# yharby/flac-raster

Measured on NVIDIA B200. Metric: encode GSamples/s (streaming tiles -> FLAC frames; decode GSamples/s reported beside it), higher is better.
Workload: dtype int32

## Files before the change

### flac_raster_b200/csrc/frb_encode.cuh

```cuda
#pragma once
#include "frb_common.cuh"

namespace frb {

constexpr int kEncThreads = 256;
constexpr int kSPT = 16;
constexpr int kMaxBlock = kEncThreads * kSPT;
constexpr int kMaxOrd = 12;
constexpr int kMaxPO = 8;
#define PX(i) ((i) + ((uint32_t)(i) >> 4))
constexpr int kBufWords = kMaxBlock + kMaxBlock / 16;

struct EncSrc {
    const void *audio;
    uint32_t a16;
};
__device__ __forceinline__ const void *audio_at(const EncSrc &S, int64_t idx) {
    return reinterpret_cast<const uint8_t *>(S.audio) + idx * (S.a16 ? 2 : 4);
}
struct TaskLoc {
    uint32_t n, a16;
    const void *src;
};
__device__ __forceinline__ int32_t sample_at(const TaskLoc &L, uint32_t i) {
// ... 1218 lines not shown
        if (h_n_samples[i] == 0) return FRB_ERR_INVALID_ARG;
        EncStreamDev d;
        d.n_samples = h_n_samples[i]; d.audio_base = h_audio_base[i]; d.out_offset = 0;
        d.sample_rate = h_sample_rate[i]; d.frame_base = (uint32_t)frames;
        d.n_frames = (uint32_t)((h_n_samples[i] + p->blocksize - 1) / p->blocksize); d.pad = 0;
        frames += d.n_frames;
        hs[i] = d;
    }
    if (frames == 0 || frames * p->channels > 0x7FFFFFFFull) return FRB_ERR_INVALID_ARG;
    EncWorkspace w;
    if (enc_ws_layout(p, frames, d_workspace, &w) > workspace_bytes) return FRB_ERR_OVERFLOW;
    cudaStream_t s = (cudaStream_t)stream;
    static thread_local std::vector<float> win;
    static thread_local uint32_t win_bs = 0, win_n = 0;
    if (win_bs != p->blocksize || win_n != (uint32_t)level_cfg(p->level).windows) {
        win.assign(FRB_MAX_BLOCKSIZE, 1.0f);
        make_tukey(win.data(), (int)p->blocksize, 0.5f / (float)level_cfg(p->level).windows);
        win_bs = p->blocksize; win_n = (uint32_t)level_cfg(p->level).windows;
    }
    const bool ms = enc_mid_side(p);
    const uint32_t an_ch = ms ? 4u : p->channels;
    std::vector<EncStreamDev> vhs;
    if (ms) {
        vhs = hs;
        uint64_t cum = 0;
        for (uint32_t i = 0; i < p->n_streams; i++) { vhs[i].audio_base = (int64_t)(4 * cum); cum += hs[i].n_samples; }
        if (cum > frames * (uint64_t)p->blocksize) return FRB_ERR_INVALID_ARG;
        FRB_TRY(small_upload(w.vstreams, vhs.data(), sizeof(EncStreamDev) * vhs.size(), s));
    }
    FRB_TRY(small_upload(w.streams, hs.data(), sizeof(EncStreamDev) * hs.size(), s));
    FRB_TRY(small_upload(w.window, win.data(), sizeof(float) * FRB_MAX_BLOCKSIZE, s));
    FRB_TRY(small_fill(w.err_flag, 0u, 256, s));
    const std::vector<EncStreamDev> &ahs = ms ? vhs : hs;
    const EncStreamDev *an_streams = ms ? w.vstreams : w.streams;
    const bool a16 = (p->reserved & 1u) != 0;
    if (a16 && p->bps != 16) return FRB_ERR_INVALID_ARG;
    const EncSrc in_audio = {d_audio, a16 ? 1u : 0u};
    const EncSrc an_audio = ms ? EncSrc{w.vaudio, 0u} : in_audio;
    const uint32_t an_esz = an_audio.a16 ? 2u : 4u;
    const uint32_t side_ch = ms ? 3u : 0xFFFFFFFFu;
    uint32_t *sub_est = ms ? w.sub_est : nullptr;
    if (ms) {
        uint64_t max_n = 0;
        for (uint32_t i = 0; i < p->n_streams; i++) max_n = std::max<uint64_t>(max_n, hs[i].n_samples);
        uint32_t gx = (uint32_t)std::min<uint64_t>((max_n + 256 * 8 - 1) / (256 * 8), std::max<uint32_t>(1u, (uint32_t)kNumSMs * 16 / p->n_streams));
        if (gx < 1) gx = 1;
        k_ms_expand<<<gx * p->n_streams, 256, 0, s>>>(w.streams, w.vstreams, in_audio, w.vaudio, gx, w.err_flag);
        FRB_LAUNCH_CHECK("k_ms_expand");
    }
    const uint32_t slot_words = slot_words_for(p->blocksize, enc_slot_bps(p));
    static bool attr_set[64] = {false};
    if (first_call_on_device(attr_set)) {
        FRB_CUDA(cudaFuncSetAttribute(k_encode_subframes, cudaFuncAttributeMaxDynamicSharedMemorySize, (int)sizeof(EncShared)));
        cudaFuncSetAttribute(k_enc_code<false>, cudaFuncAttributePreferredSharedMemoryCarveout, 20);
        cudaFuncSetAttribute(k_enc_stats<false, 9>, cudaFuncAttributePreferredSharedMemoryCarveout, 5);
        cudaFuncSetAttribute(k_enc_stats<false, 13>, cudaFuncAttributePreferredSharedMemoryCarveout, 5);
        cudaFuncSetAttribute(k_enc_stats<false, 0>, cudaFuncAttributePreferredSharedMemoryCarveout, 5);
        cudaGetLastError();
    }
    const LevelCfg cfg = level_cfg(p->level);
    const bool fast = p->blocksize == (uint32_t)kMaxBlock && cfg.max_po >= 3 && cfg.max_po <= 6;
    std::vector<uint32_t> slow;
    const uint32_t total_tasks = (uint32_t)(frames * an_ch);
    if (fast) {
        const uint64_t base_addr = (uint64_t)reinterpret_cast<uintptr_t>(an_audio.audio);
        if (base_addr & (an_esz - 1)) return FRB_ERR_INVALID_ARG;
        for (uint32_t i = 0; i < p->n_streams; i++) {
            const EncStreamDev &d = ahs[i];
            const bool tail = (d.n_samples % p->blocksize) != 0;
            for (uint32_t c = 0; c < an_ch; c++) {
                const bool aligned = ((base_addr + ((uint64_t)d.audio_base + (uint64_t)c * d.n_samples) * an_esz) & (an_esz == 2 ? 7u : 15u)) == 0;
                for (uint32_t k = aligned ? (tail ? d.n_frames - 1 : d.n_frames) : 0; k < d.n_frames; k++)
                    slow.push_back((d.frame_base + k) * an_ch + c);
            }
        }
        if (!slow.empty()) {
            if (4 * slow.size() <= (1u << 20)) FRB_TRY(small_upload(w.slow_tasks, slow.data(), 4 * slow.size(), s));
            else {
                FRB_CUDA(cudaMemcpyAsync(w.slow_tasks, slow.data(), 4 * slow.size(), cudaMemcpyHostToDevice, s));
                FRB_CUDA(cudaStreamSynchronize(s));
            }
        }
    }
    k_frame_table<<<(uint32_t)((frames + 255) / 256), 256, 0, s>>>(an_streams, p->n_streams, p->blocksize, (uint32_t)frames, w.frame_table);
    FRB_LAUNCH_CHECK("k_frame_table");
    prof_begin(6, s);
    if (fast && slow.size() < total_tasks) {
        const uint32_t windows = (uint32_t)cfg.windows, max_lpc = (uint32_t)cfg.max_lpc_order;
        const uint32_t n_cands = max_lpc == 0 ? 0u : windows == 1 ? 1u : windows == 2 ? 3u : 9u;
        const bool wide = p->bps > 16;
        const dim3 grid((uint32_t)frames, ms ? 3u : p->channels), grid_side((uint32_t)frames, 1);
        prof_begin(4, s);
#define FRB_STATS(W, NL, G, C0, EX) k_enc_stats<W, NL><<<G, kEncThreads, 0, s>>>(w.frame_table, an_ch, p->bps, windows, (uint32_t)cfg.max_po, an_audio, \
            w.window, w.stats, w.autoc, w.fx_fin, C0, EX)
#define FRB_STATS_L(NL) do { if (wide) FRB_STATS(true, NL, grid, 0u, 0u); else FRB_STATS(false, NL, grid, 0u, 0u); \
                             if (ms) FRB_STATS(true, NL, grid_side, 3u, 1u); } while (0)
        if (max_lpc == 0) FRB_STATS_L(0);
        else if (max_lpc <= 8) FRB_STATS_L(9);
        else FRB_STATS_L(13);
#undef FRB_STATS_L
#undef FRB_STATS
        prof_end(4, s);
        FRB_LAUNCH_CHECK("k_enc_stats");
        k_enc_fixed<<<(total_tasks + 3) / 4, 128, 0, s>>>(w.frame_table, an_ch, p->bps, (uint32_t)cfg.max_po, total_tasks, an_audio,
                                                        w.stats, w.fx_fin, side_ch);
        FRB_LAUNCH_CHECK("k_enc_fixed");
        const uint32_t n_slots = n_cands;
        const uint32_t model_threads = total_tasks * n_slots;
        if (n_cands) {
#define FRB_MODEL(MO) k_enc_model<MO><<<(model_threads + 127) / 128, 128, 0, s>>>(w.frame_table, an_ch, p->bps, \
            p->blocksize, windows, max_lpc, n_slots, total_tasks, an_audio, w.stats, w.autoc, w.cands, side_ch)
        if (max_lpc <= 8) FRB_MODEL(8); else FRB_MODEL(12);
#undef FRB_MODEL
        FRB_LAUNCH_CHECK("k_enc_model");
        }
        prof_begin(0, s);
#define FRB_CODE(W, G, C0, EX) k_enc_code<W><<<G, kEncThreads, 0, s>>>(w.frame_table, an_ch, p->bps, (uint32_t)cfg.max_po, n_cands, an_audio, \
            w.stats, w.cands, slot_words, w.slots, w.sub_bits, C0, EX, sub_est)
        if (wide) FRB_CODE(true, grid, 0u, 0u); else FRB_CODE(false, grid, 0u, 0u);
        if (ms) FRB_CODE(true, grid_side, 3u, 1u);
#undef FRB_CODE
        prof_end(0, s);
        FRB_LAUNCH_CHECK("k_enc_code");
    }
    if (!fast || !slow.empty()) {
        const uint32_t grid = fast ? (uint32_t)slow.size() : total_tasks;
        k_encode_subframes<<<grid, kEncThreads, sizeof(EncShared), s>>>(
            an_streams, p->n_streams, an_ch, p->bps, p->blocksize, p->level, an_audio, w.window, slot_words, w.slots, w.sub_bits,
            fast ? w.slow_tasks : nullptr, side_ch, sub_est);
        FRB_LAUNCH_CHECK("k_encode_subframes");
    }
    prof_end(6, s);
    if (ms) {
        k_ms_choose<<<(uint32_t)((frames + 255) / 256), 256, 0, s>>>(w.streams, p->n_streams, p->blocksize, (uint32_t)frames,
                                                                   (uint32_t)cfg.loose, w.sub_est, w.frame_sel);
        FRB_LAUNCH_CHECK("k_ms_choose");
    }
    k_frame_sizes<<<(uint32_t)((frames + 255) / 256), 256, 0, s>>>(w.streams, p->n_streams, p->channels, p->blocksize,
                                                                 (uint32_t)frames, w.sub_bits, w.frame_bytes, an_ch, ms ? w.frame_sel : nullptr);
    FRB_LAUNCH_CHECK("k_frame_sizes");
    t_last_analyse.ws = d_workspace; t_last_analyse.frames = frames; t_last_analyse.n_streams = p->n_streams;
    k_stream_scan<<<p->n_streams, 1024, 0, s>>>(w.streams, w.frame_bytes, w.frame_off, w.stream_bytes);
    FRB_LAUNCH_CHECK("k_stream_scan");
    if (d_stream_bytes)
        FRB_CUDA(cudaMemcpyAsync(d_stream_bytes, w.stream_bytes, 8 * (size_t)p->n_streams, cudaMemcpyDeviceToDevice, s));
    if (h_stream_bytes) {
        FRB_TRY(small_download(h_stream_bytes, w.stream_bytes, 8 * (size_t)p->n_streams, s));
    }
    return FRB_OK;
}

extern "C" int frb_encode_emit(const frb_encode_params *p, void *d_workspace, size_t workspace_bytes,
                               const uint64_t *h_out_offset, uint8_t *d_out, size_t out_capacity,
                               uint32_t *d_frame_bytes, void *stream) {
    using namespace frb;
    if (!enc_params_ok(p) || !d_workspace || !d_out) return FRB_ERR_INVALID_ARG;
    cudaStream_t s = (cudaStream_t)stream;
    EncWorkspace w0;
    (void)enc_ws_layout(p, 0, d_workspace, &w0);
    uint64_t frames;
    if (t_last_analyse.ws == d_workspace && t_last_analyse.n_streams == p->n_streams && t_last_analyse.frames) frames = t_last_analyse.frames;
    else {
        EncStreamDev last;
        FRB_TRY(small_download(&last, w0.streams + (p->n_streams - 1), sizeof last, s));
        frames = (uint64_t)last.frame_base + last.n_frames;
    }
    EncWorkspace w;
    if (enc_ws_layout(p, frames, d_workspace, &w) > workspace_bytes) return FRB_ERR_OVERFLOW;
    if (h_out_offset) {
        FRB_TRY(small_upload(w.out_offs, h_out_offset, 8 * (size_t)p->n_streams, s));
        k_set_out_offsets<<<(p->n_streams + 255) / 256, 256, 0, s>>>(w.streams, w.out_offs, p->n_streams);
        FRB_LAUNCH_CHECK("k_set_out_offsets");
    } else {
// ... 50 lines not shown
```

### flac_raster_b200/csrc/frb_encode_fast.cuh

```cuda
#pragma once

constexpr int kMaxSets = 6;
constexpr int kMaxCands = 9;
constexpr int kLags = kMaxOrd + 1;

struct EncSubStats {
    unsigned long long e[5];
    uint32_t wasted, flags;
    uint32_t fx_order, fx_bits, fx_po, fx_bad;
    uint8_t fx_params[64];
};
struct EncCand {
    int32_t type, order, precision, shift;
    int32_t coefs[kMaxOrd];
};

struct FrameDesc {
    int64_t src0;
    uint64_t ns;
    uint32_t n, stream;
};
__global__ void __launch_bounds__(256)
k_frame_table(const EncStreamDev *__restrict__ streams, uint32_t n_streams, uint32_t blocksize, uint32_t total_frames,
              FrameDesc *__restrict__ out) {
// ... 152 lines not shown
        const bool hi = lane >= 16;
        const unsigned long long b_m = __shfl_sync(0xFFFFFFFFu, b, src), mine_m = __shfl_sync(0xFFFFFFFFu, mine, src);
        const uint32_t myl_m = __shfl_sync(0xFFFFFFFFu, myl, src);
        const bool act_m = (uint32_t)src < M, actd_m = act_m && myl_m <= P;
        uint32_t k1 = 0, b1 = 0, k2 = 0, b2 = 0;
        if (act_m) rice_estimate(hi ? b_m : a, (!hi && lane == 0) ? np0 - order : np0, k_limit, &k1, &b1);
        if (hi ? actd_m : act_m) {
            uint32_t np = hi ? (n >> (P - myl_m)) : np1;
            if (hi ? (((uint32_t)src >> (myl_m - 1)) == 0) : (lane == 0)) np -= order;
            rice_estimate(hi ? mine_m : a + b, np, k_limit, &k2, &b2);
        }
        const uint32_t kb_u = __shfl_sync(0xFFFFFFFFu, k1, src + 16), bb_u = __shfl_sync(0xFFFFFFFFu, b1, src + 16);
        const uint32_t kd_u = __shfl_sync(0xFFFFFFFFu, k2, src + 16), bd_u = __shfl_sync(0xFFFFFFFFu, b2, src + 16);
        if (!hi) { ka = k1; ba = b1; kb = kb_u; bb = bb_u; kc = k2; bc = b2; kd = kd_u; bd = bd_u; }
    } else {
        if (act) {
            rice_estimate(a, lane == 0 ? np0 - order : np0, k_limit, &ka, &ba);
            rice_estimate(b, np0, k_limit, &kb, &bb);
            rice_estimate(a + b, lane == 0 ? np1 - order : np1, k_limit, &kc, &bc);
        }
        if (actd) {
            uint32_t np = n >> (P - myl);
            if (((uint32_t)lane >> (myl - 1)) == 0) np -= order;
            rice_estimate(mine, np, k_limit, &kd, &bd);
        }
    }
    unsigned long long tot = warp_sum_u32((ba & 0xFFFFu) + (bb & 0xFFFFu), (ba >> 16) + (bb >> 16)) + 6;
    uint32_t rb = tot > 0xFFFFFFFFull ? 0xFFFFFFFFu : (uint32_t)tot, best_l = 0;
    tot = warp_sum_u32(bc & 0xFFFFu, bc >> 16) + 6;
    { const uint32_t c = tot > 0xFFFFFFFFull ? 0xFFFFFFFFu : (uint32_t)tot; if (c < rb) { rb = c; best_l = 1; } }
#pragma unroll
    for (int l = 2; l <= 6; l++) {
        if ((uint32_t)l <= P) {
            const uint32_t x = (actd && myl == (uint32_t)l) ? bd : 0u;
            tot = warp_sum_u32(x & 0xFFFFu, x >> 16) + 6;
            const uint32_t c = tot > 0xFFFFFFFFull ? 0xFFFFFFFFu : (uint32_t)tot;
            if (c < rb) { rb = c; best_l = (uint32_t)l; }
        }
    }
    if (best_l == 0) { if (act) { params[2 * lane] = (uint8_t)ka; params[2 * lane + 1] = (uint8_t)kb; } }
    else if (best_l == 1) { if (act) params[lane] = (uint8_t)kc; }
    else if (actd && myl == best_l) params[(uint32_t)lane >> (myl - 1)] = (uint8_t)kd;
    *rb_out = rb; *best_l_out = best_l;
}

struct StatsShared {
    uint32_t orv[8], diff[8];
    unsigned long long e[8][5];
    double ac[8][kLags];
};

#ifndef FRB_STATS_MINB
#define FRB_STATS_MINB 4
#endif
#ifndef FRB_CODE_MINB
#define FRB_CODE_MINB 4
#endif
#ifndef FRB_CODE_RELOAD
#define FRB_CODE_RELOAD 1
#endif
#ifndef FRB_STATS_LATEWIN
#define FRB_STATS_LATEWIN 0
#endif
#ifndef FRB_STATS_RELOAD
#define FRB_STATS_RELOAD 1
#endif
template <bool WIDE, int NLAGS>
__global__ void __launch_bounds__(kEncThreads, (NLAGS > 9 || WIDE) ? 2 : FRB_STATS_MINB)
k_enc_stats(const FrameDesc *__restrict__ frames, uint32_t channels, uint32_t bps_stream,
            uint32_t windows, uint32_t max_po_cfg, const EncSrc audio,
            const float *__restrict__ window, EncSubStats *__restrict__ stats, double *__restrict__ autoc_out,
            unsigned long long *__restrict__ fx_fin, uint32_t c0, uint32_t side_extra) {
    __shared__ StatsShared S;
    const uint32_t cch = blockIdx.y + c0, sbps = bps_stream + side_extra;
    const uint32_t task = blockIdx.x * channels + cch;
    const TaskLoc L = locate_task(frames, audio, blockIdx.x, cch);
    if (!fast_eligible(L)) return;
    const int tid = threadIdx.x, lane = tid & 31, warp = tid >> 5;
    constexpr uint32_t n = kMaxBlock;
    constexpr int HALO = NLAGS > 0 ? NLAGS - 1 : 0;
    int32_t xs[28];
    load_samples28(L, tid, xs);
    float wv[kSPT + HALO + 1];
    auto load_window = [&]() {
        if (NLAGS > 0) {
            const float4 *wp = reinterpret_cast<const float4 *>(window + tid * kSPT) - HALO / 4;
#pragma unroll
            for (int q = 0; q < (kSPT + HALO) / 4; q++) {
                float4 v = make_float4(0.f, 0.f, 0.f, 0.f);
                if (tid > 0 || q >= HALO / 4) v = __ldg(wp + q);
                wv[4 * q] = v.x; wv[4 * q + 1] = v.y; wv[4 * q + 2] = v.z; wv[4 * q + 3] = v.w;
            }
        }
    };
#if !FRB_STATS_LATEWIN
    load_window();
#endif
    uint32_t orv = 0, diff = 0;
    const int32_t x_first = sample_at(L, 0);
#pragma unroll
    for (int s = 0; s < kSPT; s++) { orv |= (uint32_t)xs[12 + s]; diff |= (uint32_t)(xs[12 + s] ^ x_first); }
    orv = __reduce_or_sync(0xFFFFFFFFu, orv);
    diff = __reduce_or_sync(0xFFFFFFFFu, diff);
    if (lane == 0) { S.orv[warp] = orv; S.diff[warp] = diff; }
    __syncthreads();
    orv = 0; diff = 0;
#pragma unroll
    for (int w = 0; w < 8; w++) { orv |= S.orv[w]; diff |= S.diff[w]; }
    uint32_t wasted = orv ? (uint32_t)(__ffs((int)orv) - 1) : 0;
    if (wasted > sbps) wasted = sbps;
    if (wasted) {
#pragma unroll
// ... 294 lines not shown
            er = __dadd_rn(er, __ddiv_rn((double)lpv[i], (double)(1 << ns)));
            long long q = llround(er);
            if (q > qmax) q = qmax; else if (q < qmin) q = qmin;
            er = __dsub_rn(er, (double)q); C.coefs[i] = (int32_t)q;
        }
        sh = 0;
    }
    C.type = 3; C.order = (int)order; C.precision = (int)prec; C.shift = sh;
}

template <int MAXO>
__global__ void __launch_bounds__(128)
k_enc_model(const FrameDesc *__restrict__ frames, uint32_t channels, uint32_t bps_stream,
            uint32_t blocksize, uint32_t windows, uint32_t max_lpc_cfg, uint32_t n_cands, uint32_t total_tasks,
            const EncSrc audio, EncSubStats *__restrict__ stats, const double *__restrict__ autoc_in,
            EncCand *__restrict__ cands, uint32_t side_ch) {
    const uint32_t gid = blockIdx.x * blockDim.x + threadIdx.x;
    const uint32_t task = gid / n_cands, slot = gid - task * n_cands;
    if (task >= total_tasks) return;
    const uint32_t f = task / channels;
    const TaskLoc L = locate_task(frames, audio, f, task - f * channels);
    if (!fast_eligible(L)) return;
    constexpr uint32_t n = kMaxBlock;
    EncCand C;
    C.type = 0; C.order = 0; C.precision = 0; C.shift = 0;
#pragma unroll
    for (int j = 0; j < kMaxOrd; j++) C.coefs[j] = 0;
    const EncSubStats *stp = stats + task;
    const uint32_t st_flags = stp->flags;
    const uint32_t bps = bps_stream + (task - f * channels == side_ch ? 1u : 0u) - stp->wasted;
    if (!(st_flags & 1u)) {
        if constexpr (MAXO > 0) {
            uint32_t set = 0;
            bool punch = false;
            if (slot == 0) set = 0;
            else if (slot <= 2) set = slot;
            else { const uint32_t ci = slot - 3; set = 3 + ci / 2; punch = (ci & 1u) != 0; }
            const double *a = autoc_in + ((size_t)task * kMaxSets + set) * kLags;
            double autoc[MAXO + 1];
#pragma unroll
            for (int l = 0; l <= MAXO; l++) autoc[l] = a[l];
            const uint32_t max_lpc = max_lpc_cfg;
            if (punch) {
                const double *root = autoc_in + (size_t)task * kMaxSets * kLags;
#pragma unroll
                for (int l = 0; l < MAXO; l++) if ((uint32_t)l < max_lpc) autoc[l] = root[l] - autoc[l];
            }
            model_one<MAXO>(autoc, max_lpc, n, bps, qlp_precision_for(bps_stream, blocksize), C);
        }
    }
    cands[(size_t)task * kMaxCands + slot] = C;
}

template <bool WIDE>
struct CodeShared {
    uint32_t bitbuf[WIDE ? 4232 : 2052];
    SearchShared search;
    uint8_t best_params[64];
    uint32_t scan[kEncThreads / 32];
};

__device__ __forceinline__ void put_bits_atomic(uint32_t *buf, uint32_t pos, uint32_t v, uint32_t len) {
    const uint32_t o = pos & 31u;
    const unsigned long long x = (unsigned long long)v << (64u - o - len);
    const uint32_t hi = (uint32_t)(x >> 32), lo = (uint32_t)x;
    if (hi) atomicOr(&buf[pos >> 5], hi);
    if (lo) atomicOr(&buf[(pos >> 5) + 1], lo);
}

__device__ __forceinline__ void put_sample_atomic(uint32_t *buf, uint32_t pos, int32_t x, uint32_t bps) {
    if (bps > 32) { put_bits_atomic(buf, pos, x < 0 ? 1u : 0u, bps - 32); put_bits_atomic(buf, pos + bps - 32, (uint32_t)x, 32); }
    else if (bps) put_bits_atomic(buf, pos, (uint32_t)x & (bps == 32 ? 0xFFFFFFFFu : ((1u << bps) - 1u)), bps);
}

struct PackWriter {
    uint32_t addr, fill, hi;
    __device__ __forceinline__ void init(uint32_t *b, uint32_t bitpos) {
        addr = (uint32_t)__cvta_generic_to_shared(b) + ((bitpos >> 5) << 2); fill = bitpos & 31u; hi = 0;
    }
    __device__ __forceinline__ void put(uint32_t v, uint32_t len) {
        const uint32_t vh = v << (32u - len);
        hi |= vh >> fill;
        const uint32_t lo = __funnelshift_lc(0u, vh, 32u - fill);
        fill += len;
        asm volatile("{\n\t.reg .pred p;\n\t"
                     "setp.ge.u32 p, %1, 32;\n\t"
                     "@p red.shared.or.b32 [%2], %0;\n\t"
                     "@p mov.b32 %0, %3;\n\t"
                     "@p add.u32 %2, %2, 4;\n\t"
                     "@p sub.u32 %1, %1, 32;\n\t"
                     "}\n" : "+r"(hi), "+r"(fill), "+r"(addr) : "r"(lo) : "memory");
    }
    __device__ __forceinline__ void put0(uint32_t v, uint32_t len) {
        uint32_t vh;
        asm("shl.b32 %0, %1, %2;" : "=r"(vh) : "r"(v), "r"(32u - len));
        hi |= vh >> fill;
        const uint32_t lo = __funnelshift_lc(0u, vh, 32u - fill);
        fill += len;
        asm volatile("{\n\t.reg .pred p;\n\t"
                     "setp.ge.u32 p, %1, 32;\n\t"
                     "@p red.shared.or.b32 [%2], %0;\n\t"
                     "@p mov.b32 %0, %3;\n\t"
                     "@p add.u32 %2, %2, 4;\n\t"
                     "@p sub.u32 %1, %1, 32;\n\t"
                     "}\n" : "+r"(hi), "+r"(fill), "+r"(addr) : "r"(lo) : "memory");
    }
    __device__ __forceinline__ void zeros(uint32_t q) {
        fill += q;
        while (fill >= 32) {
// ... 15 lines not shown
    const uint32_t kbit = 1u << kcur, kmask = kbit - 1u, k1 = kcur + 1;
#pragma unroll 1
    for (uint32_t s = skip; s < (uint32_t)kSPT; s++) {
        const uint32_t u = (uint32_t)r[s];
        const uint32_t q = u >> kcur;
        const uint32_t tailv = kbit | (u & kmask);
        if (q + k1 <= 32) bw.put(tailv, q + k1);
        else { bw.zeros(q); bw.put(tailv, k1); }
    }
    bw.finish();
}

template <bool WIDE, int TAPS>
__device__ __forceinline__ uint32_t residual16(const int32_t (&xs)[28], const int32_t (&cf)[kMaxOrd], int shift, int32_t (&r)[kSPT],
                                               uint32_t *hi_mismatch) {
    uint32_t ora = 0, bad = 0;
#pragma unroll
    for (int s = 0; s < kSPT; s++) {
        if (WIDE) {
            long long acc = 0;
#pragma unroll
            for (int j = 0; j < TAPS; j++) acc += (long long)cf[j] * (long long)xs[12 + s - 1 - j];
            const long long v = (long long)xs[12 + s] - (acc >> shift);
            r[s] = (int32_t)v;
            bad |= (uint32_t)((int32_t)(v >> 32) ^ (r[s] >> 31));
        } else {
            int32_t acc = 0;
#pragma unroll
            for (int j = 0; j < TAPS; j++) acc += cf[j] * xs[12 + s - 1 - j];
            r[s] = (int32_t)((uint32_t)xs[12 + s] - (uint32_t)(acc >> shift));
        }
        ora |= (uint32_t)abs(r[s]);
    }
    *hi_mismatch = bad;
    return ora;
}

__device__ __noinline__ bool residual_overflows(const void *src, uint32_t a16, uint32_t wasted, const EncCand *__restrict__ C, int tid) {
    const int order = C->order, shift = C->shift;
    TaskLoc L;
    L.src = src; L.a16 = a16; L.n = kMaxBlock;
    bool bad = false;
    for (int s = 0; s < kSPT; s++) {
        const int i = tid * kSPT + s;
        if (i < order) continue;
        long long acc = 0;
        for (int j = 0; j < order; j++) acc += (long long)C->coefs[j] * (long long)(sample_at(L, (uint32_t)(i - 1 - j)) >> wasted);
        const long long v = (long long)(sample_at(L, (uint32_t)i) >> wasted) - (acc >> shift);
        if (v > 2147483647ll || v <= -2147483648ll) bad = true;
    }
    return bad;
}

template <bool WIDE>
__global__ void __launch_bounds__(kEncThreads, WIDE ? 2 : FRB_CODE_MINB)
k_enc_code(const FrameDesc *__restrict__ frames, uint32_t channels, uint32_t bps_stream,
           uint32_t max_po_cfg, uint32_t n_cands, const EncSrc audio,
           const EncSubStats *__restrict__ stats, const EncCand *__restrict__ cands, uint32_t slot_words,
           uint32_t *__restrict__ slots, uint32_t *__restrict__ sub_bits, uint32_t c0, uint32_t side_extra,
           uint32_t *__restrict__ sub_est) {
    __shared__ __align__(16) CodeShared<WIDE> S;
    const uint32_t cch = blockIdx.y + c0;
    const uint32_t task = blockIdx.x * channels + cch;
    const TaskLoc L = locate_task(frames, audio, blockIdx.x, cch);
    if (!fast_eligible(L)) return;
    const int tid = threadIdx.x, lane = tid & 31, warp = tid >> 5;
    constexpr uint32_t n = kMaxBlock;
    const uint32_t k_limit = bps_stream > 16 ? 31u : 15u;
    const EncSubStats *stp = stats + task;
    const uint32_t wasted = stp->wasted, st_flags = stp->flags;
    const uint32_t bps = bps_stream + side_extra - wasted;
    constexpr bool RELOAD = FRB_CODE_RELOAD != 0 && !WIDE;
    int32_t xs0[28];
    if constexpr (!RELOAD) {
        load_samples28(L, tid, xs0);
        if (wasted) {
#pragma unroll
            for (int j = 0; j < 28; j++) xs0[j] >>= wasted;
        }
    }
    {
        constexpr int nq = (int)(sizeof(S.bitbuf) / 16);
        uint4 *b4 = reinterpret_cast<uint4 *>(S.bitbuf);
        for (int q = tid; q < nq; q += kEncThreads) b4[q] = make_uint4(0, 0, 0, 0);
    }
    const uint32_t verbatim_bits = 8 + wasted + n * bps;
    int best_type = 1, best_order = 0, best_prec = 0, best_shift = 0, best_slot = -1, best_po = 0;
    uint32_t best_bits = verbatim_bits;
    int32_t r[kSPT];
    int cur_slot = -1;
    const uint32_t P = max_po_cfg;

    auto eval_residual = [&](const EncCand &C, const EncCand *Cg, bool *bad_out) -> uint32_t {
        int32_t xr[28];
        if constexpr (RELOAD) {
            load_samples28(L, tid, xr);
            if (wasted) {
#pragma unroll
                for (int j = 0; j < 28; j++) xr[j] >>= wasted;
            }
        }
        const int32_t (&xs)[28] = pick_ref<RELOAD>(xr, xs0);
        int32_t cf[kMaxOrd];
#pragma unroll
        for (int j = 0; j < kMaxOrd; j++) cf[j] = C.coefs[j];
        uint32_t ora, him;
        if (C.order <= 4) ora = residual16<WIDE, 4>(xs, cf, C.shift, r, &him);
        else if (C.order <= 8) ora = residual16<WIDE, 8>(xs, cf, C.shift, r, &him);
        else ora = residual16<WIDE, 12>(xs, cf, C.shift, r, &him);
        if (tid == 0) {
            ora = 0;
#pragma unroll
            for (int s = 0; s < kSPT; s++) { if (s < C.order) r[s] = 0; ora |= (uint32_t)abs(r[s]); }
        }
        bool bad = false;
        if (Cg != nullptr && ((WIDE && him) || ora >= 0x40000000u)) bad = residual_overflows(L.src, L.a16, wasted, Cg, tid);
        *bad_out = bad;
        return ora;
    };

    if (st_flags & 1u) {
        const uint32_t b = 8 + wasted + bps;
        if (b < best_bits) { best_type = 0; best_bits = b; }
    } else {
        if ((st_flags & 2u) && stp->fx_bits < best_bits) {
            best_bits = stp->fx_bits; best_type = 2; best_order = (int)stp->fx_order; best_po = (int)stp->fx_po; best_slot = -2;
            if (tid < 64) S.best_params[tid] = stp->fx_params[tid];
        }
        for (uint32_t slot = 0; slot <= n_cands; slot++) {
            const bool final_pass = slot == n_cands;
            const EncCand *Cg = nullptr;
            EncCand C;
            if (!final_pass) {
                Cg = cands + (size_t)task * kMaxCands + slot;
                C = *Cg;
                if (C.type == 0) continue;
            } else {
                if (best_type < 2 || best_slot == cur_slot) break;
                if (best_slot == -2) {
                    C.type = 2; C.order = best_order; C.precision = 0; C.shift = 0;
#pragma unroll
                    for (int j = 0; j < kMaxOrd; j++) C.coefs[j] = 0;
                    if (best_order == 1) { C.coefs[0] = 1; }
                    else if (best_order == 2) { C.coefs[0] = 2; C.coefs[1] = -1; }
                    else if (best_order == 3) { C.coefs[0] = 3; C.coefs[1] = -3; C.coefs[2] = 1; }
                    else if (best_order == 4) { C.coefs[0] = 4; C.coefs[1] = -6; C.coefs[2] = 4; C.coefs[3] = -1; }
                } else {
                    Cg = cands + (size_t)task * kMaxCands + best_slot;
                    C = *Cg;
                }
            }
            bool bad_lane;
            const uint32_t ora = eval_residual(C, Cg, &bad_lane);
            if (final_pass) break;
            cur_slot = (int)slot;
            const uint32_t order = (uint32_t)C.order;
            unsigned long long s64;
            if (ora < 0x08000000u) {
                uint32_t s32 = 0;
#pragma unroll
                for (int s = 0; s < kSPT; s++) s32 = __sad(r[s], 0, s32);
                s64 = s32;
            } else {
                s64 = 0;
#pragma unroll
                for (int s = 0; s < kSPT; s++) s64 += (unsigned long long)(uint32_t)abs(r[s]);
            }
            finest_sums(s64, P, tid, S.search.fin);
            if (__syncthreads_or(bad_lane ? 1 : 0)) continue;
            if (warp == 0) {
                uint32_t rb, bl;
                warp_search(S.search.fin, order, P, k_limit, lane, S.search.params, &rb, &bl);
                if (lane == 0) { S.search.rb = rb; S.search.best_l = bl; }
            }
            __syncthreads();
            const uint32_t total = 8 + wasted + 4 + 5 + order * ((uint32_t)C.precision + bps) + S.search.rb;
            if (total < best_bits) {
                best_bits = total; best_type = 3; best_order = C.order; best_prec = C.precision; best_shift = C.shift;
                best_slot = (int)slot; best_po = (int)(P - S.search.best_l);
                if (tid < 64) S.best_params[tid] = S.search.params[tid];
            }
        }
    }
    __syncthreads();

    int type = best_type;
    const int order = best_order;
    uint32_t my_bits = 0, kcur = 0, plen = 4, method = 0, qmax = 0;
    bool pstart = false;
    if (type >= 2) {
        const uint32_t tl = 8 - (uint32_t)best_po;
        kcur = S.best_params[(uint32_t)tid >> tl];
        if (WIDE) {
            const uint32_t cnt = 1u << best_po;
            method = __syncthreads_or(((uint32_t)tid < cnt && S.best_params[tid < 64 ? tid : 0] >= 15) ? 1 : 0) ? 1u : 0u;
        }
        plen = method ? 5u : 4u;
        pstart = ((uint32_t)tid & ((1u << tl) - 1u)) == 0;
        uint32_t qsum = 0;
#pragma unroll
        for (int s = 0; s < kSPT; s++) { r[s] = (int32_t)zigzag(r[s]); const uint32_t q = (uint32_t)r[s] >> kcur; qsum += q; qmax = max(qmax, q); }
        const uint32_t cnt = tid == 0 ? kSPT - (uint32_t)order : (uint32_t)kSPT;
        my_bits = qsum + cnt * (1 + kcur) + (pstart ? plen : 0u);
    }
    uint32_t hdr_bits = 8 + wasted;
    if (type == 0) hdr_bits += bps;
    else if (type == 2) hdr_bits += (uint32_t)order * bps + 6;
    else if (type == 3) hdr_bits += (uint32_t)order * bps + 9 + (uint32_t)(order * best_prec) + 6;
    uint32_t total_res, my_off;
    {
        uint32_t inc = my_bits;
#pragma unroll
        for (int o = 1; o < 32; o <<= 1) { const uint32_t t = __shfl_up_sync(0xFFFFFFFFu, inc, o); if (lane >= o) inc += t; }
        if (lane == 31) S.scan[warp] = inc;
        __syncthreads();
        uint32_t base = 0, tot = 0;
#pragma unroll
        for (int w = 0; w < kEncThreads / 32; w++) { const uint32_t s = S.scan[w]; if (w < warp) base += s; tot += s; }
        total_res = tot; my_off = base + inc - my_bits;
    }
    if (type >= 2 && hdr_bits + total_res > verbatim_bits) type = 1;
    uint32_t total_bits;
    if (type == 1) { hdr_bits = 8 + wasted; total_bits = verbatim_bits; }
    else total_bits = hdr_bits + total_res;

    const uint32_t mask_bps = bps >= 32 ? 0xFFFFFFFFu : ((1u << bps) - 1u);
    const uint32_t pos0 = 8 + wasted;
    if (tid == 0) {
        const uint32_t typecode = type == 0 ? 0u : type == 1 ? 1u : type == 2 ? (8u | (uint32_t)order) : (32u | (uint32_t)(order - 1));
        put_bits_atomic(S.bitbuf, 0, (typecode << 1) | (wasted ? 1u : 0u), 8);
        if (wasted) put_bits_atomic(S.bitbuf, 8 + wasted - 1, 1, 1);
        if (type == 0 && bps) put_sample_atomic(S.bitbuf, pos0, sample_at(L, 0) >> wasted, bps);
    }
    if (type >= 2) {
        if (tid >= 32 && tid < 32 + order)
            put_sample_atomic(S.bitbuf, pos0 + (uint32_t)(tid - 32) * bps, sample_at(L, (uint32_t)(tid - 32)) >> wasted, bps);
        const uint32_t pos1 = pos0 + (uint32_t)order * bps;
        if (type == 3) {
            const uint32_t prec = (uint32_t)best_prec;
            if (tid == 96) put_bits_atomic(S.bitbuf, pos1, ((prec - 1) << 5) | ((uint32_t)best_shift & 31u), 9);
            if (tid >= 64 && tid < 64 + order)
                put_bits_atomic(S.bitbuf, pos1 + 9 + (uint32_t)(tid - 64) * prec,
                                (uint32_t)cands[(size_t)task * kMaxCands + best_slot].coefs[tid - 64] & ((1u << prec) - 1u), prec);
        }
        if (tid == 128) put_bits_atomic(S.bitbuf, hdr_bits - 6, (method << 4) | (uint32_t)best_po, 6);
    }
    PackWriter bw;
    if (type == 1) {
        bw.init(S.bitbuf, hdr_bits + (uint32_t)tid * kSPT * bps);
        if (bps) {
            int32_t xr[28];
            if constexpr (RELOAD) {
                load_samples28(L, tid, xr);
#pragma unroll
                for (int j = 12; j < 28; j++) xr[j] >>= wasted;
            }
            const int32_t (&xs)[28] = pick_ref<RELOAD>(xr, xs0);
            if (WIDE && bps > 32) {
#pragma unroll
                for (int s = 0; s < kSPT; s++) { bw.put(xs[12 + s] < 0 ? 1u : 0u, bps - 32); bw.put((uint32_t)xs[12 + s], 32); }
            } else {
#pragma unroll
                for (int s = 0; s < kSPT; s++) bw.put((uint32_t)xs[12 + s] & mask_bps, bps);
            }
        }
        bw.finish();
    } else if (type >= 2) {
        bw.init(S.bitbuf, hdr_bits + my_off);
        if (pstart) bw.put(kcur, plen);
        const uint32_t kbit = 1u << kcur, kmask = kbit - 1u, k1 = kcur + 1;
        const uint32_t skip = tid == 0 ? (uint32_t)order : 0u;
        if (qmax + k1 <= 32) {
#pragma unroll
            for (int s = 0; s < kSPT; s++) {
                const uint32_t u = (uint32_t)r[s];
                const uint32_t q = u >> kcur;
                const uint32_t tailv = kbit | (u & kmask);
                if (s < kMaxOrd) { const bool on = (uint32_t)s >= skip; bw.put0(on ? tailv : 0u, on ? q + k1 : 0u); }
                else bw.put(tailv, q + k1);
            }
            bw.finish();
        } else {
            pack_codes_long(bw.addr, bw.fill, bw.hi, kcur, skip, r[0], r[1], r[2], r[3], r[4], r[5], r[6], r[7], r[8], r[9], r[10], r[11],
                            r[12], r[13], r[14], r[15]);
        }
    }
    __syncthreads();
    const uint32_t nwords = (total_bits + 31) / 32;
    uint32_t *slot = slots + (size_t)task * slot_words;
    const uint32_t nq = (nwords + 1 + 3) / 4;
    const uint4 *b4 = reinterpret_cast<const uint4 *>(S.bitbuf);
    uint4 *s4 = reinterpret_cast<uint4 *>(slot);
    for (uint32_t q = tid; q < nq && q * 4 < slot_words; q += kEncThreads) s4[q] = b4[q];
    if (tid == 0) { sub_bits[task] = total_bits; if (sub_est) sub_est[task] = best_bits; }
}
```

Baseline: 111.6.

## Add warp-per-subframe 16-bit code kernel replacing block-per-subframe path

```diff
diff --git a/flac_raster_b200/csrc/frb_encode.cuh b/flac_raster_b200/csrc/frb_encode.cuh
--- a/flac_raster_b200/csrc/frb_encode.cuh
+++ b/flac_raster_b200/csrc/frb_encode.cuh
@@ -1294,7 +1294,7 @@
     static bool attr_set[64] = {false};
     if (first_call_on_device(attr_set)) {
         FRB_CUDA(cudaFuncSetAttribute(k_encode_subframes, cudaFuncAttributeMaxDynamicSharedMemorySize, (int)sizeof(EncShared)));
-        cudaFuncSetAttribute(k_enc_code<false>, cudaFuncAttributePreferredSharedMemoryCarveout, 20);
+        cudaFuncSetAttribute(k_enc_code16, cudaFuncAttributePreferredSharedMemoryCarveout, 100);
         cudaFuncSetAttribute(k_enc_stats<false, 9>, cudaFuncAttributePreferredSharedMemoryCarveout, 5);
         cudaFuncSetAttribute(k_enc_stats<false, 13>, cudaFuncAttributePreferredSharedMemoryCarveout, 5);
         cudaFuncSetAttribute(k_enc_stats<false, 0>, cudaFuncAttributePreferredSharedMemoryCarveout, 5);
@@ -1357,10 +1357,16 @@
         FRB_LAUNCH_CHECK("k_enc_model");
         }
         prof_begin(0, s);
-#define FRB_CODE(W, G, C0, EX) k_enc_code<W><<<G, kEncThreads, 0, s>>>(w.frame_table, an_ch, p->bps, (uint32_t)cfg.max_po, n_cands, an_audio, \
+#define FRB_CODE(G, C0, EX) k_enc_code<<<G, kEncThreads, 0, s>>>(w.frame_table, an_ch, p->bps, (uint32_t)cfg.max_po, n_cands, an_audio, \
             w.stats, w.cands, slot_words, w.slots, w.sub_bits, C0, EX, sub_est)
-        if (wide) FRB_CODE(true, grid, 0u, 0u); else FRB_CODE(false, grid, 0u, 0u);
-        if (ms) FRB_CODE(true, grid_side, 3u, 1u);
+        if (wide) FRB_CODE(grid, 0u, 0u);
+        else {
+            const uint64_t warps = frames * (uint64_t)grid.y;
+            k_enc_code16<<<(uint32_t)((warps + kCode16Warps - 1) / kCode16Warps), kCode16Warps * 32, 0, s>>>(
+                w.frame_table, an_ch, grid.y, (uint32_t)frames, p->bps, (uint32_t)cfg.max_po, n_cands, an_audio, w.stats, w.cands,
+                slot_words, w.slots, w.sub_bits, sub_est);
+        }
+        if (ms) FRB_CODE(grid_side, 3u, 1u);
 #undef FRB_CODE
         prof_end(0, s);
         FRB_LAUNCH_CHECK("k_enc_code");
diff --git a/flac_raster_b200/csrc/frb_encode_fast.cuh b/flac_raster_b200/csrc/frb_encode_fast.cuh
--- a/flac_raster_b200/csrc/frb_encode_fast.cuh
+++ b/flac_raster_b200/csrc/frb_encode_fast.cuh
@@ -228,12 +228,6 @@
 
 #ifndef FRB_STATS_MINB
 #define FRB_STATS_MINB 4
-#endif
-#ifndef FRB_CODE_MINB
-#define FRB_CODE_MINB 4
-#endif
-#ifndef FRB_CODE_RELOAD
-#define FRB_CODE_RELOAD 1
 #endif
 #ifndef FRB_STATS_LATEWIN
 #define FRB_STATS_LATEWIN 0
@@ -634,9 +628,8 @@
     cands[(size_t)task * kMaxCands + slot] = C;
 }
 
-template <bool WIDE>
 struct CodeShared {
-    uint32_t bitbuf[WIDE ? 4232 : 2052];
+    uint32_t bitbuf[4232];
     SearchShared search;
     uint8_t best_params[64];
     uint32_t scan[kEncThreads / 32];
@@ -758,14 +751,13 @@
     return bad;
 }
 
-template <bool WIDE>
-__global__ void __launch_bounds__(kEncThreads, WIDE ? 2 : FRB_CODE_MINB)
+__global__ void __launch_bounds__(kEncThreads, 2)
 k_enc_code(const FrameDesc *__restrict__ frames, uint32_t channels, uint32_t bps_stream,
            uint32_t max_po_cfg, uint32_t n_cands, const EncSrc audio,
            const EncSubStats *__restrict__ stats, const EncCand *__restrict__ cands, uint32_t slot_words,
            uint32_t *__restrict__ slots, uint32_t *__restrict__ sub_bits, uint32_t c0, uint32_t side_extra,
            uint32_t *__restrict__ sub_est) {
-    __shared__ __align__(16) CodeShared<WIDE> S;
+    __shared__ __align__(16) CodeShared S;
     const uint32_t cch = blockIdx.y + c0;
     const uint32_t task = blockIdx.x * channels + cch;
     const TaskLoc L = locate_task(frames, audio, blockIdx.x, cch);
@@ -776,14 +768,11 @@
     const EncSubStats *stp = stats + task;
     const uint32_t wasted = stp->wasted, st_flags = stp->flags;
     const uint32_t bps = bps_stream + side_extra - wasted;
-    constexpr bool RELOAD = FRB_CODE_RELOAD != 0 && !WIDE;
-    int32_t xs0[28];
-    if constexpr (!RELOAD) {
-        load_samples28(L, tid, xs0);
-        if (wasted) {
-#pragma unroll
-            for (int j = 0; j < 28; j++) xs0[j] >>= wasted;
-        }
+    int32_t xs[28];
+    load_samples28(L, tid, xs);
+    if (wasted) {
+#pragma unroll
+        for (int j = 0; j < 28; j++) xs[j] >>= wasted;
     }
     {
         constexpr int nq = (int)(sizeof(S.bitbuf) / 16);
@@ -798,29 +787,20 @@
     const uint32_t P = max_po_cfg;
 
     auto eval_residual = [&](const EncCand &C, const EncCand *Cg, bool *bad_out) -> uint32_t {
-        int32_t xr[28];
-        if constexpr (RELOAD) {
-            load_samples28(L, tid, xr);
-            if (wasted) {
-#pragma unroll
-                for (int j = 0; j < 28; j++) xr[j] >>= wasted;
-            }
-        }
-        const int32_t (&xs)[28] = pick_ref<RELOAD>(xr, xs0);
         int32_t cf[kMaxOrd];
 #pragma unroll
         for (int j = 0; j < kMaxOrd; j++) cf[j] = C.coefs[j];
         uint32_t ora, him;
-        if (C.order <= 4) ora = residual16<WIDE, 4>(xs, cf, C.shift, r, &him);
-        else if (C.order <= 8) ora = residual16<WIDE, 8>(xs, cf, C.shift, r, &him);
-        else ora = residual16<WIDE, 12>(xs, cf, C.shift, r, &him);
+        if (C.order <= 4) ora = residual16<true, 4>(xs, cf, C.shift, r, &him);
+        else if (C.order <= 8) ora = residual16<true, 8>(xs, cf, C.shift, r, &him);
+        else ora = residual16<true, 12>(xs, cf, C.shift, r, &him);
         if (tid == 0) {
             ora = 0;
 #pragma unroll
             for (int s = 0; s < kSPT; s++) { if (s < C.order) r[s] = 0; ora |= (uint32_t)abs(r[s]); }
         }
         bool bad = false;
-        if (Cg != nullptr && ((WIDE && him) || ora >= 0x40000000u)) bad = residual_overflows(L.src, L.a16, wasted, Cg, tid);
+        if (Cg != nullptr && (him || ora >= 0x40000000u)) bad = residual_overflows(L.src, L.a16, wasted, Cg, tid);
         *bad_out = bad;
         return ora;
     };
@@ -897,7 +877,7 @@
     if (type >= 2) {
         const uint32_t tl = 8 - (uint32_t)best_po;
         kcur = S.best_params[(uint32_t)tid >> tl];
-        if (WIDE) {
+        {
             const uint32_t cnt = 1u << best_po;
             method = __syncthreads_or(((uint32_t)tid < cnt && S.best_params[tid < 64 ? tid : 0] >= 15) ? 1 : 0) ? 1u : 0u;
         }
@@ -955,14 +935,7 @@
     if (type == 1) {
         bw.init(S.bitbuf, hdr_bits + (uint32_t)tid * kSPT * bps);
         if (bps) {
-            int32_t xr[28];
-            if constexpr (RELOAD) {
-                load_samples28(L, tid, xr);
-#pragma unroll
-                for (int j = 12; j < 28; j++) xr[j] >>= wasted;
-            }
-            const int32_t (&xs)[28] = pick_ref<RELOAD>(xr, xs0);
-            if (WIDE && bps > 32) {
+            if (bps > 32) {
 #pragma unroll
                 for (int s = 0; s < kSPT; s++) { bw.put(xs[12 + s] < 0 ? 1u : 0u, bps - 32); bw.put((uint32_t)xs[12 + s], 32); }
             } else {
@@ -1000,3 +973,257 @@
     for (uint32_t q = tid; q < nq && q * 4 < slot_words; q += kEncThreads) s4[q] = b4[q];
     if (tid == 0) { sub_bits[task] = total_bits; if (sub_est) sub_est[task] = best_bits; }
 }
+
+#ifndef FRB_CODE16_WARPS
+#define FRB_CODE16_WARPS 4
+#endif
+#ifndef FRB_CODE16_MINB
+#define FRB_CODE16_MINB 6
+#endif
+constexpr int kCode16Warps = FRB_CODE16_WARPS;
+struct Code16Shared {
+    uint32_t bitbuf[2052];
+    unsigned long long fin[64];
+    uint8_t params[64], best_params[64];
+};
+
+__global__ void __launch_bounds__(kCode16Warps * 32, FRB_CODE16_MINB)
+k_enc_code16(const FrameDesc *__restrict__ frames, uint32_t channels, uint32_t nch, uint32_t n_frames, uint32_t bps_stream,
+             uint32_t max_po_cfg, uint32_t n_cands, const EncSrc audio,
+             const EncSubStats *__restrict__ stats, const EncCand *__restrict__ cands, uint32_t slot_words,
+             uint32_t *__restrict__ slots, uint32_t *__restrict__ sub_bits, uint32_t *__restrict__ sub_est) {
+    __shared__ __align__(16) Code16Shared SW[kCode16Warps];
+    const int lane = threadIdx.x & 31;
+    Code16Shared &S = SW[threadIdx.x >> 5];
+    const uint32_t g = blockIdx.x * kCode16Warps + (threadIdx.x >> 5);
+    const uint32_t f = g / nch, cch = g - f * nch;
+    if (f >= n_frames) return;
+    const uint32_t task = f * channels + cch;
+    const TaskLoc L = locate_task(frames, audio, f, cch);
+    if (!fast_eligible(L)) return;
+    constexpr uint32_t n = kMaxBlock, k_limit = 15;
+    const EncSubStats *stp = stats + task;
+    const uint32_t wasted = stp->wasted, st_flags = stp->flags;
+    const uint32_t bps = bps_stream - wasted;
+    uint4 *b4 = reinterpret_cast<uint4 *>(S.bitbuf);
+    auto zero_buf = [&]() {
+        constexpr int nq = (int)(sizeof(S.bitbuf) / 16);
+        for (int q = lane; q < nq; q += 32) b4[q] = make_uint4(0, 0, 0, 0);
+        __syncwarp();
+    };
+    auto zero_words = [&](uint32_t a, uint32_t b) {
+        for (uint32_t w = a + lane; w < b; w += 32) S.bitbuf[w] = 0;
+    };
+    const uint32_t verbatim_bits = 8 + wasted + n * bps;
+    int best_type = 1, best_order = 0, best_prec = 0, best_shift = 0, best_slot = -1, best_po = 0;
+    uint32_t best_bits = verbatim_bits;
+    const uint32_t P = max_po_cfg;
+    int type = 1;
+    uint32_t hdr_bits = 8 + wasted, total_res = 0;
+    int cached_slot = -1;
+    uint32_t cleared = 0;
+
+    if (st_flags & 1u) {
+        const uint32_t b = 8 + wasted + bps;
+        if (b < best_bits) { best_type = 0; best_bits = b; }
+    } else {
+        if ((st_flags & 2u) && stp->fx_bits < best_bits) {
+            best_bits = stp->fx_bits; best_type = 2; best_order = (int)stp->fx_order; best_po = (int)stp->fx_po; best_slot = -2;
+            S.best_params[lane] = stp->fx_params[lane]; S.best_params[lane + 32] = stp->fx_params[lane + 32];
+        }
+        for (uint32_t slot = 0; slot <= n_cands; slot++) {
+            const bool final_pass = slot == n_cands;
+            const EncCand *Cg = cands + (size_t)task * kMaxCands + slot;
+            EncCand C;
+            if (!final_pass) {
+                C = *Cg;
+                if (C.type == 0) continue;
+            } else {
+                if (best_type < 2) break;
+                if (best_slot == -2) {
+                    C.type = 2; C.order = best_order; C.precision = 0; C.shift = 0;
+#pragma unroll
+                    for (int j = 0; j < kMaxOrd; j++) C.coefs[j] = 0;
+                    if (best_order == 1) { C.coefs[0] = 1; }
+                    else if (best_order == 2) { C.coefs[0] = 2; C.coefs[1] = -1; }
+                    else if (best_order == 3) { C.coefs[0] = 3; C.coefs[1] = -3; C.coefs[2] = 1; }
+                    else if (best_order == 4) { C.coefs[0] = 4; C.coefs[1] = -6; C.coefs[2] = 4; C.coefs[3] = -1; }
+                } else C = cands[(size_t)task * kMaxCands + best_slot];
+                type = best_type;
+                hdr_bits += (uint32_t)best_order * bps + 6 + (type == 3 ? 9 + (uint32_t)(best_order * best_prec) : 0u);
+                __syncwarp();
+            }
+            int32_t cf[kMaxOrd];
+#pragma unroll
+            for (int j = 0; j < kMaxOrd; j++) cf[j] = C.coefs[j];
+            const uint32_t order = (uint32_t)C.order;
+            const uint32_t tl = 8 - (uint32_t)best_po;
+            const bool use_cache = final_pass && best_slot == cached_slot;
+            bool bad = false;
+            uint32_t zor = 0;
+            for (int c = 0; c < 8; c++) {
+                const int vt = 32 * c + lane;
+                uint4 *cache = b4 + 1 + 64 * c + 2 * lane;
+                int32_t r[kSPT];
+                uint32_t ora = 0;
+                if (use_cache && cleared <= 4 + 256u * (uint32_t)c) {
+                    const uint4 a = cache[0], b = cache[1];
+                    const uint32_t w[8] = {a.x, a.y, a.z, a.w, b.x, b.y, b.z, b.w};
+#pragma unroll
+                    for (int s = 0; s < 8; s++) { r[2 * s] = (int32_t)(w[s] & 0xFFFFu); r[2 * s + 1] = (int32_t)(w[s] >> 16); }
+                } else {
+                    int32_t xs[28];
+                    load_samples28(L, vt, xs);
+                    if (wasted) {
+#pragma unroll
+                        for (int j = 0; j < 28; j++) xs[j] >>= wasted;
+                    }
+                    uint32_t him;
+                    if (order <= 4) ora = residual16<false, 4>(xs, cf, C.shift, r, &him);
+                    else if (order <= 8) ora = residual16<false, 8>(xs, cf, C.shift, r, &him);
+                    else ora = residual16<false, 12>(xs, cf, C.shift, r, &him);
+                    if (vt == 0) {
+                        ora = 0;
+#pragma unroll
+                        for (int s = 0; s < kSPT; s++) { if ((uint32_t)s < order) r[s] = 0; ora |= (uint32_t)abs(r[s]); }
+                    }
+                    if (final_pass) {
+#pragma unroll
+                        for (int s = 0; s < kSPT; s++) r[s] = (int32_t)zigzag(r[s]);
+                    }
+                }
+                if (!final_pass) {
+                    if (ora >= 0x40000000u) bad |= residual_overflows(L.src, L.a16, wasted, Cg, vt);
+                    unsigned long long s64;
+                    if (ora < 0x08000000u) {
+                        uint32_t s32 = 0;
+#pragma unroll
+                        for (int s = 0; s < kSPT; s++) s32 = __sad(r[s], 0, s32);
+                        s64 = s32;
+                    } else {
+                        s64 = 0;
+#pragma unroll
+                        for (int s = 0; s < kSPT; s++) s64 += (unsigned long long)(uint32_t)abs(r[s]);
+                    }
+                    finest_sums(s64, P, vt, S.fin);
+                    uint32_t w[8];
+#pragma unroll
+                    for (int s = 0; s < 8; s++) {
+                        const uint32_t z0 = zigzag(r[2 * s]), z1 = zigzag(r[2 * s + 1]);
+                        zor |= z0 | z1;
+                        w[s] = z0 | (z1 << 16);
+                    }
+                    cache[0] = make_uint4(w[0], w[1], w[2], w[3]);
+                    cache[1] = make_uint4(w[4], w[5], w[6], w[7]);
+                    continue;
+                }
+                const uint32_t kcur = S.best_params[(uint32_t)vt >> tl];
+                const bool pstart = ((uint32_t)vt & ((1u << tl) - 1u)) == 0;
+                uint32_t qsum = 0, qmax = 0;
+#pragma unroll
+                for (int s = 0; s < kSPT; s++) { const uint32_t q = (uint32_t)r[s] >> kcur; qsum += q; qmax = max(qmax, q); }
+                const uint32_t cnt = vt == 0 ? kSPT - order : (uint32_t)kSPT;
+                const uint32_t my_bits = qsum + cnt * (1 + kcur) + (pstart ? 4u : 0u);
+                uint32_t inc = my_bits;
+#pragma unroll
+                for (int o = 1; o < 32; o <<= 1) { const uint32_t t = __shfl_up_sync(0xFFFFFFFFu, inc, o); if (lane >= o) inc += t; }
+                const uint32_t chunk_bits = __shfl_sync(0xFFFFFFFFu, inc, 31);
+                if (hdr_bits + total_res + chunk_bits > verbatim_bits) { type = 1; break; }
+                {
+                    const uint32_t end = (hdr_bits + total_res + chunk_bits + 31) / 32;
+                    __syncwarp();
+                    zero_words(cleared, end);
+                    cleared = max(cleared, end);
+                    __syncwarp();
+                }
+                PackWriter bw;
+                bw.init(S.bitbuf, hdr_bits + total_res + inc - my_bits);
+                total_res += chunk_bits;
+                if (pstart) bw.put(kcur, 4);
+                const uint32_t kbit = 1u << kcur, kmask = kbit - 1u, k1 = kcur + 1;
+                const uint32_t skip = vt == 0 ? order : 0u;
+                if (qmax + k1 <= 32) {
+#pragma unroll
+                    for (int s = 0; s < kSPT; s++) {
+                        const uint32_t u = (uint32_t)r[s];
+                        const uint32_t q = u >> kcur;
+                        const uint32_t tailv = kbit | (u & kmask);
+                        if (s < kMaxOrd) { const bool on = (uint32_t)s >= skip; bw.put0(on ? tailv : 0u, on ? q + k1 : 0u); }
+                        else bw.put(tailv, q + k1);
+                    }
+                    bw.finish();
+                } else {
+                    pack_codes_long(bw.addr, bw.fill, bw.hi, kcur, skip, r[0], r[1], r[2], r[3], r[4], r[5], r[6], r[7], r[8], r[9], r[10],
+                                    r[11], r[12], r[13], r[14], r[15]);
+                }
+            }
+            if (final_pass) break;
+            cached_slot = __any_sync(0xFFFFFFFFu, zor >> 16) ? -1 : (int)slot;
+            if (__any_sync(0xFFFFFFFFu, bad)) continue;
+            __syncwarp();
+            uint32_t rb, bl;
+            warp_search(S.fin, order, P, k_limit, lane, S.params, &rb, &bl);
+            __syncwarp();
+            const uint32_t total = 8 + wasted + 4 + 5 + order * ((uint32_t)C.precision + bps) + rb;
+            if (total < best_bits) {
+                best_bits = total; best_type = 3; best_order = C.order; best_prec = C.precision; best_shift = C.shift;
+                best_slot = (int)slot; best_po = (int)(P - bl);
+                S.best_params[lane] = S.params[lane]; S.best_params[lane + 32] = S.params[lane + 32];
+            }
+        }
+    }
+    const int order = best_order;
+    uint32_t total_bits;
+    if (best_type == 0) type = 0;
+    if (type < 2) {
+        hdr_bits = 8 + wasted + (type == 0 ? bps : 0u);
+        total_bits = type == 0 ? hdr_bits : verbatim_bits;
+        __syncwarp();
+        zero_buf();
+    } else {
+        total_bits = hdr_bits + total_res;
+        zero_words(cleared, 4 * (((total_bits + 31) / 32 + 1 + 3) / 4));
+        __syncwarp();
+    }
+
+    const uint32_t pos0 = 8 + wasted;
+    if (lane == 0) {
+        const uint32_t typecode = type == 0 ? 0u : type == 1 ? 1u : type == 2 ? (8u | (uint32_t)order) : (32u | (uint32_t)(order - 1));
+        put_bits_atomic(S.bitbuf, 0, (typecode << 1) | (wasted ? 1u : 0u), 8);
+        if (wasted) put_bits_atomic(S.bitbuf, 8 + wasted - 1, 1, 1);
+        if (type == 0 && bps) put_sample_atomic(S.bitbuf, pos0, sample_at(L, 0) >> wasted, bps);
+    }
+    if (type >= 2) {
+        const uint32_t pos1 = pos0 + (uint32_t)order * bps;
+        if (lane < order) {
+            put_sample_atomic(S.bitbuf, pos0 + (uint32_t)lane * bps, sample_at(L, (uint32_t)lane) >> wasted, bps);
+            if (type == 3) {
+                const uint32_t prec = (uint32_t)best_prec;
+                put_bits_atomic(S.bitbuf, pos1 + 9 + (uint32_t)lane * prec,
+                                (uint32_t)cands[(size_t)task * kMaxCands + best_slot].coefs[lane] & ((1u << prec) - 1u), prec);
+            }
+        }
+        if (type == 3 && lane == 31) put_bits_atomic(S.bitbuf, pos1, (((uint32_t)best_prec - 1) << 5) | ((uint32_t)best_shift & 31u), 9);
+        if (lane == 30) put_bits_atomic(S.bitbuf, hdr_bits - 6, (uint32_t)best_po, 6);
+    }
+    if (type == 1 && bps) {
+        const uint32_t mask_bps = (1u << bps) - 1u;
+        for (int c = 0; c < 8; c++) {
+            const int vt = 32 * c + lane;
+            int32_t xs[28];
+            load_samples28(L, vt, xs);
+            PackWriter bw;
+            bw.init(S.bitbuf, hdr_bits + (uint32_t)vt * kSPT * bps);
+#pragma unroll
+            for (int s = 0; s < kSPT; s++) bw.put((uint32_t)(xs[12 + s] >> wasted) & mask_bps, bps);
+            bw.finish();
+        }
+    }
+    __syncwarp();
+    const uint32_t nwords = (total_bits + 31) / 32;
+    uint32_t *slot = slots + (size_t)task * slot_words;
+    const uint32_t nq = (nwords + 1 + 3) / 4;
+    uint4 *s4 = reinterpret_cast<uint4 *>(slot);
+    for (uint32_t q = lane; q < nq && q * 4 < slot_words; q += 32) s4[q] = b4[q];
+    if (lane == 0) { sub_bits[task] = total_bits; if (sub_est) sub_est[task] = best_bits; }
+}
```

Result: no change. 112.7 (median of 6 runs) (+1.0%).
